# treangenlab/bronko

Hardware: AMD Instinct MI355X
Metric: reads/sec through call k-mer->pileup, SARS-CoV-2 k=21 (higher is better)
Workload: dtype u64

## Files before the change

bronko_amd/csrc/bk_finalize_lean.hip:

```cpp
#include <hip/hip_runtime.h>

#include "bk_device.h"
#include "bk_kernels.h"
#include "bk_scan_common.h"
#include "bk_finalize_common.h"

namespace bk {

constexpr int kLeanVBlock = 1024;
constexpr uint32_t kLeanVq = 64;
constexpr uint32_t kLeanWin = 256;

__device__ __forceinline__ void lean_vote(unsigned int* cnt, unsigned int* mxv, uint32_t span, uint32_t p0, const FinalizeArgs& a, uint32_t cell,
                                          uint32_t idx, bool canonical, uint64_t c, uint32_t isrc, int k, uint32_t v) {
    uint32_t bit_idx;
    bool forward;
    if (canonical) { bit_idx = ((uint32_t)(c >> (2 * idx)) & 3u) ^ 3u; forward = isrc != 0; }
    else { bit_idx = (uint32_t)(c >> (2 * (k - 1 - (int)idx))) & 3u; forward = isrc == 0; }
    const uint32_t pos = cell - p0;
    if (cell >= p0 && pos < span) {
        const uint32_t at = ((forward ? 0u : 4u) + bit_idx) * span + pos;
        __hip_atomic_fetch_add(cnt + at, 1u, __ATOMIC_RELAXED, __HIP_MEMORY_SCOPE_WORKGROUP);
        __hip_atomic_fetch_max(mxv + at, v, __ATOMIC_RELAXED, __HIP_MEMORY_SCOPE_WORKGROUP);
    } else {
        const size_t pc = (size_t)cell * 4 + bit_idx;
        atomicAdd(a.pileup + (forward ? 2 : 3) * a.plane + pc, 1ull);
        atomicMax(a.pileup + (forward ? 0 : 1) * a.plane + pc, (unsigned long long)v);
    }
}
__device__ __forceinline__ void lean_flush(const unsigned int* cnt, const unsigned int* mxv, uint32_t span, uint32_t p0, const FinalizeArgs& a) {
    for (uint32_t i = threadIdx.x; i < 8u * span; i += blockDim.x) {
        const unsigned int nv = cnt[i];
        if (!nv) continue;
        const uint32_t row = i / span, pos = i - row * span;
        const size_t pc = ((size_t)p0 + pos) * 4 + (row & 3u);
        atomicAdd(a.pileup + (row < 4u ? 2 : 3) * a.plane + pc, (unsigned long long)nv);
        atomicMax(a.pileup + (row < 4u ? 0 : 1) * a.plane + pc, (unsigned long long)mxv[i]);
    }
}

template <bool FUSED>
__global__ __launch_bounds__(kLeanVBlock) void finalize_vbin_kernel(FinalizeArgs a) {
    __shared__ unsigned int cnt[8 * kLeanWin], mxv[8 * kLeanWin];
    __shared__ uint32_t lstats[3 + 2];
    __shared__ unsigned int tmask[kLeanVq * kVRowsPerPos / 32 + 1];
    extern __shared__ __attribute__((aligned(16))) unsigned int acc[];
    const IndexView& ix = a.ix;
    const int k = ix.k;
    const uint32_t span = (uint32_t)ix.v_span, rl = span + 1u;
    const uint32_t q0 = blockIdx.x * kLeanVq;
    const uint32_t nq = ix.n_full + span;
    const uint32_t id_lo = min(q0 >= span - 1u ? q0 - (span - 1u) : 0u, ix.n_full - 1u);
    const uint32_t p0 = ix.id_rec[id_lo].cell;
    for (uint32_t i = threadIdx.x; i < 8u * kLeanWin; i += kLeanVBlock) { cnt[i] = 0u; mxv[i] = 0u; }
    if (threadIdx.x < 5) lstats[threadIdx.x] = 0u;
    if constexpr (FUSED) {
        const uint32_t n_eb = a.f_ig.n_ebins, n_bins = n_eb + a.f_ig.n_vbins, bin = n_eb + blockIdx.x, cap = a.f_ig.cap_v, G = a.f_ig.grid_max;
        const uint32_t upb = cap / 8u;
        const uint32_t vsize = kLeanVq * kVRowsPerPos * rl;
        const uint32_t n_units = a.f_n_wg * upb;
        const unsigned short* const bin_items = a.f_items + (size_t)n_eb * G * a.f_ig.cap_e + (size_t)blockIdx.x * G * cap;
        const bool mine = threadIdx.x < n_units;
        const uint32_t wg0 = mine ? threadIdx.x / upb : 0u, un0 = threadIdx.x - wg0 * upb;
        uint32_t hdr0 = 0u;
        uint4 v0 = make_uint4(0u, 0u, 0u, 0u);
        if (mine) { hdr0 = a.f_tab[(size_t)bin * G + wg0]; v0 = reinterpret_cast<const uint4*>(bin_items + (size_t)wg0 * cap)[un0]; }
        const unsigned long long ov_all = a.f_ov_n[a.f_ov_par];
        if (threadIdx.x <= kLeanVq * kVRowsPerPos / 32) {
            unsigned int* tw = a.f_touch + (size_t)blockIdx.x * (kLeanVq * kVRowsPerPos / 32) + threadIdx.x;
            unsigned int m = 0u;
            if (threadIdx.x < kLeanVq * kVRowsPerPos / 32) { m = *tw; if (m) *tw = 0u; }
            else m = ov_all > (unsigned long long)a.f_ov_cap ? 1u : 0u;
            tmask[threadIdx.x] = m;
        }
        for (uint32_t i = threadIdx.x; i < vsize; i += kLeanVBlock) acc[i] = 0u;
        __syncthreads();
        auto take = [&](uint32_t it) __attribute__((always_inline)) {
            __hip_atomic_fetch_add(acc + (it & 0x7fffu), (it & 0x8000u) ? 0u - 1u : 1u, __ATOMIC_RELAXED, __HIP_MEMORY_SCOPE_WORKGROUP);
        };
        auto take8 = [&](const uint4& v, uint32_t left) __attribute__((always_inline)) {
            if (left > 0u) take(v.x & 0xffffu);
            if (left > 1u) take(v.x >> 16);
            if (left > 2u) take(v.y & 0xffffu);
            if (left > 3u) take(v.y >> 16);
            if (left > 4u) take(v.z & 0xffffu);
            if (left > 5u) take(v.z >> 16);
            if (left > 6u) take(v.w & 0xffffu);
            if (left > 7u) take(v.w >> 16);
        };
        for (uint32_t u = threadIdx.x; u < n_units; u += kLeanVBlock) {
            const uint32_t wg = u / upb, un = u - wg * upb;
            uint32_t n_all; uint4 v;
            if (u == threadIdx.x) { n_all = hdr0; v = v0; }
            else { n_all = a.f_tab[(size_t)bin * G + wg]; v = reinterpret_cast<const uint4*>(bin_items + (size_t)wg * cap)[un]; }
            const uint32_t n = min(n_all, cap);
            take8(v, n > 8u * un ? n - 8u * un : 0u);
            const uint32_t g = min(n_all - n, kItemGCap);
            if (g) {
                const uint4* q = reinterpret_cast<const uint4*>(a.f_gext + ((size_t)wg * n_bins + bin) * kItemGCap);
                for (uint32_t i0 = 8u * un; i0 < g; i0 += 8u * upb * 4u) {
                    uint4 e[4];
#pragma unroll
                    for (uint32_t j = 0; j < 4u; ++j) e[j] = i0 + 8u * upb * j < g ? q[(i0 >> 3) + upb * j] : make_uint4(0u, 0u, 0u, 0u);
#pragma unroll
                    for (uint32_t j = 0; j < 4u; ++j) take8(e[j], g > i0 + 8u * upb * j ? g - i0 - 8u * upb * j : 0u);
                }
            }
        }
        {
            const uint32_t n_ov = (uint32_t)(ov_all < (unsigned long long)a.f_ov_cap ? ov_all : (unsigned long long)a.f_ov_cap);
            for (uint32_t i = threadIdx.x; i < n_ov; i += kLeanVBlock) {
                const uint32_t e = a.f_ov[i];
                if ((e >> 16) == bin) take(e & 0xffffu);
            }
        }
    }
    __syncthreads();
    unsigned long long* __restrict__ vc = const_cast<unsigned long long*>(a.counters) + ix.v_off;
    const uint32_t lpr = span, gpw = 64u / lpr;
    const uint32_t lane64 = threadIdx.x & 63u, wave = threadIdx.x >> 6;
    const uint32_t grp = lane64 / lpr, oo = lane64 - grp * lpr;
    const bool lane_on = grp < gpw;
    unsigned int kept = 0, distinct = 0, variant = 0;
    for (uint32_t g0 = 0; g0 < kLeanVq * kVRowsPerPos; g0 += (kLeanVBlock / 64) * gpw) {
        const uint32_t g = g0 + wave * gpw + grp;
        const uint32_t q = q0 + g / kVRowsPerPos, r6 = g % kVRowsPerPos;
        const bool in_row = lane_on && g < kLeanVq * kVRowsPerPos && q < nq;
        const size_t at = ((size_t)q * kVRowsPerPos + r6) * rl + oo;
        unsigned long long n;
        if constexpr (FUSED) {
            const uint32_t gg = in_row ? g : 0u;
            n = in_row ? (unsigned long long)(long long)(int32_t)acc[gg * rl + oo] : 0ull;
            if (in_row && (tmask[kLeanVq * kVRowsPerPos / 32] || ((tmask[gg >> 5] >> (gg & 31u)) & 1u))) {
                const unsigned long long pv = vc[at];
                if (pv) { n += pv; vc[at] = 0ull; }
            }
        } else {
            n = in_row ? vc[at] : 0ull;
            if (a.clear_v && n) vc[at] = 0ull;
        }
        const uint32_t d = r6 & 1u, alt = r6 >> 1;
        const bool inq = in_row && q >= oo && q - oo < ix.n_full;
        const uint32_t p = inq ? q - oo : 0u;
        const uint4 idr = *reinterpret_cast<const uint4*>(ix.id_rec + p);
        const uint64_t kmer_p = (uint64_t)idr.x | ((uint64_t)idr.y << 32);
        const uint32_t ambp = idr.w;
        const int o = (int)oo + ix.v_omin;
        if (!__ballot(n + (1ull << 26) >= (1ull << 27))) {
            int m = (int)(unsigned int)n;
#pragma unroll
            for (int off = 1; off < 32; off <<= 1) {
                const int t = __shfl_up(m, off, 64);
                if (oo >= (uint32_t)off) m += t;
            }
            n = (unsigned long long)(long long)m;
        } else {
#pragma unroll
            for (int off = 1; off < 32; off <<= 1) {
                const unsigned long long t = __shfl_up(n, off, 64);
                if (oo >= (uint32_t)off) n += t;
            }
        }
        bool act = inq && n != 0;
        const uint32_t rcid = (ambp >> 1) & 1u;
        const int j = rcid ? k - 1 - o : o;
        const int sh = 2 * (k - 1 - (act ? j : 0));
        const uint32_t bb = ((uint32_t)(kmer_p >> sh) & 3u) ^ (alt + 1u);
        const uint32_t isrc = d ^ rcid;
        const uint64_t c = (kmer_p & ~(3ull << sh)) | ((uint64_t)bb << sh);
        const uint64_t rc = revcomp_kmer(c, k);
        if (act && !(j >= ix.wstart && j < ix.wstart + ix.W && c < rc)) act = false;
        if (act) { distinct += 1; if (n < a.ci || n > a.cx) act = false; else kept += 1; }
        const uint32_t v = (uint32_t)(n > a.cs ? a.cs : n);
        bool defer = false;
        if (act) {
            bool plain = (ambp & kIdSimple) != 0u;
            if (plain && (ambp & 1u)) {
                const uint2 ans = *reinterpret_cast<const uint2*>(ix.dirty_ans + ans_index(p, (uint32_t)o, rcid ? 3u - bb : bb, k));
                plain = !(ans.y & (kAnsNone | kAnsMulti));
            }
            if (!plain) { defer = true; act = false; }
        }
        {
            const unsigned long long dm = __ballot(defer);
            if (dm) {
                unsigned int base = 0;
                if (lane64 == (uint32_t)__builtin_ctzll(dm)) base = atomicAdd(a.n_deferred, (unsigned int)__popcll(dm));
                base = (unsigned int)__shfl((int)base, __builtin_ctzll(dm));
                if (defer) {
                    const unsigned int slot = base + (unsigned int)__popcll(dm & ((1ull << lane64) - 1ull));
                    a.deferred[slot] = (uint32_t)at;
                    if (a.deferred_n) a.deferred_n[slot] = n;
                }
            }
        }
        if (act) lean_vote(cnt, mxv, kLeanWin, p0, a, idr.z + (uint32_t)j, (uint32_t)j, rcid != 0u, c, isrc, k, v);
        variant += act ? 1u : 0u;
    }
#pragma unroll
    for (int off = 32; off; off >>= 1) variant += (unsigned int)__shfl_xor((int)variant, off);
    if (lane64 == 0 && variant) atomicAdd(&lstats[1], variant);
    {
        const uint32_t W = (uint32_t)ix.W;
        const uint32_t sub = threadIdx.x & 15u, id = q0 + (threadIdx.x >> 4);
        unsigned int perfect = 0;
        if (id < ix.n_full) {
            const uint4 idr = *reinterpret_cast<const uint4*>(ix.id_rec + id);
            const unsigned long long n0 = a.counters[2 * (size_t)id], n1 = a.counters[2 * (size_t)id + 1];
            if (!(idr.w & kIdSimple)) {
                if (sub == 0u && (n0 | n1)) a.lean_e_list[atomicAdd(a.lean_n_list + 2, 1u)] = id;
            } else {
                const uint64_t km = (uint64_t)idr.x | ((uint64_t)idr.y << 32);
                const uint32_t rcid = (idr.w >> 1) & 1u;
#pragma unroll
                for (uint32_t isrc = 0; isrc < 2u; ++isrc) {
                    const unsigned long long n = isrc ? n1 : n0;
                    if (sub == 0u) distinct += n != 0;
                    if (n == 0 || n < a.ci || n > a.cx) continue;
                    if (sub == 0u) { kept += 1; perfect += 1; }
                    const uint32_t v = (uint32_t)(n > a.cs ? a.cs : n);
                    for (uint32_t t = sub; t < W; t += 16u) {
                        const uint32_t j = (uint32_t)ix.wstart + t;
                        lean_vote(cnt, mxv, kLeanWin, p0, a, idr.z + j, j, rcid != 0u, km, isrc, k, v);
                    }
                }
            }
        }
#pragma unroll
        for (int off = 32; off; off >>= 1) perfect += (unsigned int)__shfl_xor((int)perfect, off);
        if (lane64 == 0 && perfect) { atomicAdd(&lstats[0], perfect); atomicAdd(&lstats[2], perfect); }
    }
    __syncthreads();
    lean_flush(cnt, mxv, kLeanWin, p0, a);
    finalize_epilogue(a, lstats, kept, distinct, lstats + 3, (int)blockIdx.x);
}

bool finalize_lean_ok(const FinalizeArgs& a) {
    return !a.no_lean && a.lean_e_list && a.lean_n_list && !a.ix.slot_files && a.mode == 0 && !a.v_list && !a.p_list && !a.e_list && !a.ktab_keys && a.ix.n_prows == 0 && a.ix.n_u == a.ix.n_full &&
           a.ix.n_full > 0 && a.ix.n_files == 1 && a.ix.dirty_ans && a.ix.W > 1 && a.ix.v_span > 0 && a.ix.v_span <= 32 && a.partials && a.cs < (1ull << 32) &&
           a.elem_lo == 0 && a.elem_hi >= a.ix.v_off + v_plane_len(a.ix.n_full, a.ix.v_span, 0);
}
unsigned launch_finalize_lean_variant(const FinalizeArgs& a, hipStream_t stream) {
    const unsigned grid = (unsigned)((a.ix.n_full + (uint32_t)a.ix.v_span + kLeanVq - 1) / kLeanVq);
    if (a.f_items) {
        const size_t lds = (size_t)kLeanVq * kVRowsPerPos * ((size_t)a.ix.v_span + 1u) * sizeof(unsigned int);
        (void)raise_lds_limit(reinterpret_cast<const void*>(finalize_vbin_kernel<true>), lds + 20u * 1024u);
        hipLaunchKernelGGL(finalize_vbin_kernel<true>, dim3(grid), dim3(kLeanVBlock), lds, stream, a);
    } else {
        hipLaunchKernelGGL(finalize_vbin_kernel<false>, dim3(grid), dim3(kLeanVBlock), 0, stream, a);
    }
    return grid;
}
}
```

bronko_amd/csrc/bk_kernels.h:

```cpp
#pragma once
#include <hip/hip_runtime.h>

#include "../../include/bronko_hip.h"
#include "bk_device.h"

namespace bk {

struct ItemGeom {
    uint32_t n_ebins, n_vbins;
    uint32_t cap_e, cap_v;
    uint32_t vq_log2;
    uint32_t wg_items;
    uint32_t wg_stride;
    uint32_t grid_max;
};
constexpr uint32_t kEBinLog2 = 7;
constexpr uint32_t kERunMax = 255;
constexpr uint32_t kEBinSpan = (1u << kEBinLog2) + kERunMax;
constexpr uint32_t kItemGCap = 256;

struct ScanArgs {
    const IndexView* ixp;
    int32_t k, wstart, W, v_omin, v_span;
    uint64_t v_off;
// ... 21 lines not shown
    uint64_t n_records;
    const unsigned long long* n_records_dev;
    uint32_t stride_words;
    unsigned long long* counters;
    unsigned int* slabs;
    unsigned int* n_bits;
    unsigned int* n_any;
    unsigned int* l2_bits;
    unsigned int* l2_any;
    unsigned int* l2_plan;
    uint32_t l2_min_grid;
    uint2* l2_diag;
    uint32_t l2_words;
    uint32_t n_lds_bins;
    uint32_t win_lo;
    const uint32_t* win_dev;
    const uint32_t* occ;
    int32_t win_file, n_files;
    int ref_in_lds;
    unsigned long long* kmer_total;
    unsigned long long* ktab_keys;
    unsigned int* ktab_cnt;
    uint32_t ktab_log2;
    unsigned long long* ktab_overflow;
    uint32_t mate;
    unsigned int* touch_v;
    unsigned int* touch_b;
    unsigned int* touch_p;
    unsigned int* touch_e;
    unsigned long long rl_recip;
    ItemGeom ig;
    unsigned short* items;
    unsigned short* tab;
    unsigned short* gext;
    unsigned int* ov;
    unsigned long long* ov_n;
    uint32_t ov_cap;
    uint32_t ov_par;
    int n_direct;
    uint32_t stage_off;
    int ablate;
    unsigned long long* dbg;
};

struct FinalizeArgs {
    IndexView ix;
    const unsigned long long* counters;
    uint64_t elem_lo, elem_hi;
    unsigned long long ci, cs, cx;
    unsigned long long* pileup;
    size_t plane;
    unsigned long long* stats;
    unsigned char* present;
    unsigned long long* kept_total;
    unsigned long long* distinct_total;
    unsigned int* partials;
    int row_exact, row_general;
    const uint32_t* file_cell_lo;
    uint32_t max_file_cells;
    unsigned int* deferred;
    unsigned long long* deferred_n;
    int clear_v;
    unsigned int* deferred_mask;
    unsigned int* n_deferred;
    unsigned long long* ktab_keys;
    unsigned int* ktab_cnt;
    uint32_t ktab_log2;
    unsigned long long* ktab_overflow;
    uint32_t mate;
    const unsigned int* v_list;
    const unsigned int* p_list;
    const unsigned int* e_list;
    const unsigned int* n_list;
    int mode;
    const int* sel;
    int sel_file;
    unsigned int* lean_e_list;
    unsigned int* lean_n_list;
    int no_lean;
    const unsigned int* tail_e_list;
    const unsigned int* tail_n_list;
    unsigned long long* zero_e;
    size_t zero_e_n;
    int gather;
    int gather_ablate;
    unsigned long long* alias_hits;
    unsigned int* n_alias_hits;
    unsigned int alias_cap;
    const uint64_t* merged_slots;
    uint32_t n_merged_slots;
    const unsigned short* f_items;
    const unsigned short* f_tab;
    const unsigned short* f_gext;
    const unsigned int* f_ov;
    const unsigned long long* f_ov_n;
    uint32_t f_ov_cap, f_ov_par, f_n_wg;
    ItemGeom f_ig;
    unsigned int* f_touch;
};

struct FoldArgs {
    const unsigned int* slabs;
    uint32_t n_slabs;
    uint32_t n_lds_bins;
    const uint32_t* id_at;
    uint32_t win_lo;
    const uint32_t* win_dev;
    unsigned int* touch_e;
    const uint32_t* cell_codes;
    unsigned long long* counters;
};

struct PackArgs {
    const uint8_t* bases;
    uint32_t shift;
    const unsigned long long* offsets;
    uint64_t n_reads;
    int32_t k;
    uint32_t stride_words;
    uint32_t* words;
    uint16_t* lens;
    uint64_t cap;
    unsigned long long* n_records;
    unsigned long long* n_real;
    uint32_t* work;
};
struct QualArgs {
    const uint8_t* quals;
    uint32_t shift;
    uint32_t thr;
};
void launch_pack_reads(const PackArgs& a, unsigned long long* tally, hipStream_t stream, const QualArgs* q = nullptr, uint8_t* ends = nullptr);

constexpr uint32_t kEndFirst = 1u, kEndLast = 2u;
constexpr uint32_t kPrimerMinLen = BK_PRIMER_MIN_LEN, kPrimerMaxLen = BK_PRIMER_MAX_LEN, kMaxPrimers = BK_MAX_PRIMERS, kMaxPrimerMismatches = BK_PRIMER_MAX_MISMATCHES;
constexpr uint32_t kPrimerEntryWords = 9;
struct TrimArgs {
    uint32_t* words;
    uint16_t* lens;
    const uint8_t* ends;
    uint64_t n_records;
    const unsigned long long* n_records_dev;
    uint32_t stride_words;
    int32_t k;
    const uint32_t* table;
    uint32_t n_primers;
    uint32_t max_mismatches;
    unsigned long long* stats;
    unsigned long long* n_real;
};
void launch_primer_trim(const TrimArgs& a, int n_cus, hipStream_t stream);

constexpr uint32_t kAdapterMinLen = BK_ADAPTER_MIN_LEN, kAdapterMaxLen = BK_ADAPTER_MAX_LEN, kMaxAdapters = BK_MAX_ADAPTERS,
                   kAdapterMinOverlap = BK_ADAPTER_MIN_OVERLAP;
constexpr double kAdapterMaxErrorRate = BK_ADAPTER_MAX_ERROR_RATE;
static_assert(kAdapterMaxLen == 64 && kMaxAdapters <= 8, "AdapterEntry holds 64 bases, AdapterArgs eight entries");
constexpr uint32_t kNoCut = 0xFFFFFFFFu;
struct AdapterEntry {
    uint32_t code[4];
    uint32_t mask[4];
    uint32_t len;
    uint32_t allowed;
};
struct AdapterArgs {
    uint32_t* words;
    uint16_t* lens;
// ... 165 lines not shown
```

bronko_amd/csrc/bk_kernels.hip:

```cpp
#include <hip/hip_runtime.h>

#include <algorithm>
#include <cstdlib>
#include <mutex>
#include <utility>
#include <vector>

#include "bk_device.h"
#include "bk_kernels.h"
#include "bk_scan_common.h"
#include "bk_finalize_common.h"

namespace bk {


__device__ __forceinline__ int probe_table(const TableSlot* __restrict__ sub, uint32_t log2s, uint64_t key) {
    const uint32_t smask = (1u << log2s) - 1u;
    uint32_t h = hash_key(key, log2s);
    for (;;) {
        const uint4 e = *reinterpret_cast<const uint4*>(sub + h);
        const uint64_t kk = (uint64_t)e.x | ((uint64_t)e.y << 32);
        if (kk == key) return (int)e.z;
        if (kk == kEmptyKey) return -1;
        h = (h + 1) & smask;
// ... 1734 lines not shown
__global__ __launch_bounds__(256) void fold_kernel(FoldArgs f) {
    const uint64_t tid = (uint64_t)blockIdx.x * 256 + threadIdx.x;
    const uint64_t nthreads = (uint64_t)gridDim.x * 256;
    const uint32_t per = (f.n_slabs + gridDim.y - 1) / gridDim.y;
    const uint32_t b0 = blockIdx.y * per, b1 = min(f.n_slabs, b0 + per);
    for (uint64_t i = tid; i < f.n_lds_bins && b0 < b1; i += nthreads) {
        unsigned long long s0 = 0, s1 = 0;
        for (uint32_t b = b0; b < b1; ++b) {
            const unsigned int v = f.slabs[(size_t)b * f.n_lds_bins + i];
            s0 += v & 0xffffu;
            s1 += v >> 16;
        }
        if (s0 | s1) {
            const uint64_t cell = (f.win_dev ? f.win_dev[1] : f.win_lo) + i;
            const uint32_t id = f.id_at[cell];
            const uint32_t rc = ((f.cell_codes[cell >> 4] >> (2 * (cell & 15))) & 3u) == 2u ? 1u : 0u;
            touch(f.touch_e, id);
            if (s0) atomicAdd(f.counters + 2 * (size_t)id + rc, s0);
            if (s1) atomicAdd(f.counters + 2 * (size_t)id + (1u - rc), s1);
        }
    }
}

void launch_fold(const FoldArgs& f, hipStream_t stream) {
    const uint64_t work = f.n_lds_bins;
    if (work == 0) return;
    uint64_t blocks = (work + 255) / 256;
    if (blocks > 1024) blocks = 1024;
    const unsigned groups = std::max(1u, std::min(8u, f.n_slabs / 8));
    hipLaunchKernelGGL(fold_kernel, dim3((unsigned)blocks, groups), dim3(256), 0, stream, f);
}

__device__ __forceinline__ uint32_t first_of_file(const DevEntry* __restrict__ ent, uint32_t cnt, int file) {
    uint32_t lo = 0, hi = cnt;
    while (lo < hi) {
        const uint32_t mid = (lo + hi) >> 1;
        if ((int)ent[mid].file < file) lo = mid + 1; else hi = mid;
    }
    return lo;
}

template <int B>
__device__ __forceinline__ void write_lane(int& acc, int nb) { asm("v_writelane_b32 %0, %1, %2" : "+v"(acc) : "s"(nb), "n"(B)); }
template <int... B>
__device__ __forceinline__ void tally_word(uint32_t wd, int& acc, std::integer_sequence<int, B...>) {
    (write_lane<B>(acc, __popcll(__ballot((wd & (1u << B)) != 0u))), ...);
}
template <bool ATOMIC, uint32_t COL = 1u>
__device__ __forceinline__ void tally_files(const uint4& fb, uint32_t* lstats, uint32_t lane, uint32_t n_files) {
    if (!__ballot(files_any(fb))) return;
#pragma unroll
    for (uint32_t w = 0; w < 4u; ++w) {
        const uint32_t wd = w == 0u ? fb.x : w == 1u ? fb.y : w == 2u ? fb.z : fb.w;
        if (w * 32u >= n_files || !__ballot(wd != 0u)) continue;
        int acc = 0;
        tally_word(wd, acc, std::make_integer_sequence<int, 32>{});
        const uint32_t f = w * 32u + lane;
        if (lane < 32u && acc && f < n_files) {
            if (ATOMIC) atomicAdd(&lstats[f * 3u + COL], (uint32_t)acc); else lstats[f * 3u + COL] += (uint32_t)acc;
        }
    }
}

__global__ __launch_bounds__(256) void finalize_reduce_kernel(FinalizeArgs a, int n_rows, unsigned long long* zero_p, size_t zero_n) {
    __shared__ unsigned long long wave_sums[4];
    const int n3 = a.ix.n_files * 3, cols = n3 + 2;
    for (size_t i = (size_t)blockIdx.x * 256 + threadIdx.x; i < zero_n; i += (size_t)gridDim.x * 256) zero_p[i] = 0ull;
    if (a.lean_n_list && blockIdx.x == 0 && threadIdx.x < 8) a.lean_n_list[threadIdx.x] = 0u;
    const int col = blockIdx.x;
    unsigned long long s = 0;
    for (int r = threadIdx.x; r < n_rows; r += 256) s += a.partials[(size_t)r * cols + col];
#pragma unroll
    for (int off = 32; off; off >>= 1) s += __shfl_xor(s, off);
    if ((threadIdx.x & 63) == 0) wave_sums[threadIdx.x >> 6] = s;
    __syncthreads();
    if (threadIdx.x != 0) return;
    s = wave_sums[0] + wave_sums[1] + wave_sums[2] + wave_sums[3];
    if (!s) return;
    if (col < n3) { a.stats[col] += s; if (col % 3 != 2) a.present[col / 3] = 1; }
    else if (col == n3) { if (a.kept_total) *a.kept_total += s; }
    else if (a.distinct_total) *a.distinct_total += s;
}

constexpr int kVoteSlots = 512;
constexpr uint32_t kVoteMaxEntries = 4;
constexpr size_t kVoteLdsBytes = (size_t)kVoteSlots * (8 + 8 + 4 + 2) + 16;
struct VoteTable {
    unsigned long long* keys;
    unsigned long long* mx;
    unsigned int* cnt;
    unsigned int* n_used;
    unsigned short* used;
};
__device__ __forceinline__ VoteTable vt_make(unsigned char* lds) {
    VoteTable vt;
    vt.keys = reinterpret_cast<unsigned long long*>(lds);
    vt.mx = vt.keys + kVoteSlots;
    vt.cnt = reinterpret_cast<unsigned int*>(vt.mx + kVoteSlots);
    vt.n_used = vt.cnt + kVoteSlots;
    vt.used = reinterpret_cast<unsigned short*>(vt.n_used + 4);
    return vt;
}
__device__ __forceinline__ void vt_clear(const VoteTable& vt) {
    for (int i = threadIdx.x; i < kVoteSlots; i += blockDim.x) { vt.keys[i] = ~0ull; vt.mx[i] = 0ull; vt.cnt[i] = 0u; }
    if (threadIdx.x == 0) { vt.n_used[0] = 0u; vt.n_used[1] = 0u; }
}
__device__ __forceinline__ void vt_vote(const VoteTable& vt, uint32_t par, const FinalizeArgs& a, const DevEntry& e, uint64_t c, uint32_t isrc,
                                        int k, unsigned long long v) {
    if (a.mode == 1 || (a.mode == 2 && (int)e.file != a.sel_file)) return;
    uint32_t bit_idx;
    bool forward;
    if (e.canonical) { bit_idx = ((uint32_t)(c >> (2 * e.idx)) & 3u) ^ 3u; forward = isrc != 0; }
    else { bit_idx = (uint32_t)(c >> (2 * (k - 1 - e.idx))) & 3u; forward = isrc == 0; }
    const unsigned long long key = (((unsigned long long)e.cell * 4 + bit_idx) << 1) | (forward ? 0ull : 1ull);
    uint32_t h = (uint32_t)((key * 0x9E3779B97F4A7C15ull) >> 55) & (kVoteSlots - 1);
    for (int probe = 0; probe < 8; ++probe) {
        const unsigned long long old = atomicCAS(&vt.keys[h], ~0ull, key);
        if (old == ~0ull) vt.used[atomicAdd(vt.n_used + par, 1u)] = (unsigned short)h;
        if (old == ~0ull || old == key) { atomicAdd(&vt.cnt[h], 1u); atomicMax(&vt.mx[h], v); return; }
        h = (h + 1) & (kVoteSlots - 1);
    }
    vote(a, e, c, isrc, k, v);
}
__device__ __forceinline__ void vt_flush(const VoteTable& vt, uint32_t par, const FinalizeArgs& a) {
    __syncthreads();
    const unsigned int nu = vt.n_used[par];
    if (threadIdx.x == 0) vt.n_used[par ^ 1u] = 0u;
    for (unsigned int u = threadIdx.x; u < nu; u += blockDim.x) {
        const int i = vt.used[u];
        const unsigned long long key = vt.keys[i];
        const size_t cell = (size_t)(key >> 1);
        atomicAdd(a.pileup + ((key & 1ull) ? 3 : 2) * a.plane + cell, (unsigned long long)vt.cnt[i]);
        atomicMax(a.pileup + ((key & 1ull) ? 1 : 0) * a.plane + cell, vt.mx[i]);
        vt.keys[i] = ~0ull; vt.mx[i] = 0ull; vt.cnt[i] = 0u;
    }
    __syncthreads();
    if (threadIdx.x == 0) { vt.n_used[0] = 0u; vt.n_used[1] = 0u; }
}

__device__ __forceinline__ void v_kmer_of_counter(const IndexView& ix, const unsigned long long* __restrict__ vc, uint64_t vi,
                                                  uint32_t& p, uint32_t& t, uint64_t& c, uint32_t& isrc, unsigned long long& n) {
    const int k = ix.k;
    const uint64_t real_len = v_real_len(ix.n_full, ix.v_span);
    uint32_t bb;
    if (vi < real_len) {
        const uint32_t rl = (uint32_t)ix.v_span + 1u;
        const uint64_t row = vi / rl;
        const uint32_t oo = (uint32_t)(vi % rl);
        n = 0;
        if (vc) for (uint32_t x = 0; x <= oo; ++x) n += vc[row * rl + x];
        const uint32_t r6 = (uint32_t)(row % kVRowsPerPos);
        p = (uint32_t)(row / kVRowsPerPos) - oo;
        const uint32_t rcid = (ix.amb[p] >> 1) & 1u;
        const int o = (int)oo + ix.v_omin;
        const int j = rcid ? k - 1 - o : o;
        const uint32_t own = (uint32_t)(ix.kmer_of[p] >> (2 * (k - 1 - j))) & 3u;
        bb = own ^ ((r6 >> 1) + 1u);
        isrc = (r6 & 1u) ^ rcid;
        t = (uint32_t)(j - ix.wstart);
    } else {
        const uint64_t x = vi - real_len;
        isrc = (uint32_t)x & 1u;
        bb = (uint32_t)(x >> 1) & 3u;
        p = ix.prow_id[x >> 3];
        t = ix.prow_t[x >> 3];
        n = vc ? vc[vi] : 0ull;
// ... 662 lines not shown
            v = v > a.cs ? a.cs : v;

            int s = -1;
            if (lane < ix.W) {
                if (ci < n_e) {
                    s = (int)ix.slot_of[(size_t)(ci >> 1) * ix.W + lane];
                } else {
                    const int sh = 2 * (k - 1 - (ix.wstart + lane));
                    s = probe_table(ix.table + (size_t)lane * S, ix.log2s, c & ~(3ull << sh));
                }
            }
            if (a.mode == 1) note_alias(s, c, isrc, v);
            for (unsigned long long bm = __ballot(s >= 0); bm; bm &= bm - 1ull) {
                const int sb = __shfl(s, __builtin_ctzll(bm));
                const uint32_t off = ix.ent_off[sb], cnt = ix.ent_len[sb];
                for (uint32_t q = (uint32_t)lane; q < cnt; q += 64u) {
                    const DevEntry e = ix.entries[off + q];
                    if (atomicAdd(&hits[e.file], 1u) == 0u) touched[atomicAdd(ntouched, 1u)] = e.file;
                    vote(a, e, c, isrc, k, v);
                }
            }
            __syncthreads();
            const uint32_t nt = *ntouched;
            uint32_t n_perfect = 0;
            int my_perfect = -1;
            for (uint32_t q = lane; q < ((nt + 63u) & ~63u); q += 64) {
                bool perfect = false;
                if (q < nt) {
                    const uint32_t g = touched[q];
                    const uint32_t h = hits[g];
                    hits[g] = 0;
                    perfect = h == (uint32_t)ix.W;
                    if (do_stats) lstats[g * 3 + (perfect ? 0 : 1)] += 1;
                    if (perfect) my_perfect = (int)g;
                }
                n_perfect += (uint32_t)__popcll(__ballot(perfect));
            }
            if (do_stats && n_perfect == 1 && my_perfect >= 0) lstats[my_perfect * 3 + 2] += 1;
            __syncthreads();
            if (lane == 0) *ntouched = 0;
            __syncthreads();
        }
    };
    if (a.mode == 1 && ix.ent_files) {
        for (uint64_t item0 = (uint64_t)blockIdx.x * 64; item0 < n_items; item0 += (uint64_t)gridDim.x * 64) {
            const uint64_t item = item0 + (uint32_t)lane;
            const bool on = item < n_items;
            unsigned long long v = 0;
            uint64_t c = 0;
            uint32_t isrc = 0, p_ = 0, t_ = 0;
            if (on) v_kmer_of_counter(ix, nullptr, a.deferred[item], p_, t_, c, isrc, v);
            uint4 acc = make_uint4(0u, 0u, 0u, 0u);
            uint32_t found = 0, alias_n = 0;
            int alias_sb = -1;
            bool generic = false;
            for (int t = 0; t < ix.W; ++t) {
                const int sh = 2 * (k - 1 - (ix.wstart + t));
                const int sb = on ? probe_table(ix.table + (size_t)t * S, ix.log2s, c & ~(3ull << sh)) : -1;
                if (sb < 0) continue;
                const uint4 fb = ix.ent_files[sb];
                generic |= !files_any(fb);
                acc.x |= fb.x; acc.y |= fb.y; acc.z |= fb.z; acc.w |= fb.w;
                found |= 1u << t;
                alias_sb = (a.alias_hits && ix.slot_alias && ((ix.slot_alias[(uint32_t)sb >> 5] >> ((uint32_t)sb & 31u)) & 1u)) ? (alias_n++ ? -2 : sb) : alias_sb;
            }
            generic |= found == 0xffffffffu >> (32 - ix.W);
            generic |= alias_sb == -2;
            if (on && !generic && alias_sb >= 0) {
                unsigned long long n_; uint64_t c2; uint32_t i2, p2, t2;
                v_kmer_of_counter(ix, a.counters + ix.v_off, a.deferred[item], p2, t2, c2, i2, n_);
                note_alias(alias_sb, c, isrc, n_);
            }
            if (on && a.deferred_mask) a.deferred_mask[item] = found;
            if (!on || generic) acc = make_uint4(0u, 0u, 0u, 0u);
            tally_files<false>(acc, lstats, (uint32_t)lane, (uint32_t)ix.n_files);
            for (unsigned long long gm = __ballot(on && generic); gm; gm &= gm - 1ull) wave_item(item0 + (uint64_t)__builtin_ctzll(gm));
        }
    } else
    for (uint64_t item = blockIdx.x; item < n_items + n_tail; item += gridDim.x) wave_item(item);
    __syncthreads();
    if (lane == 0) { ntouched[0] = 0; ntouched[1] = 0; }
    __syncthreads();
    if (do_stats) finalize_epilogue(a, lstats, tail_kept, tail_distinct, ntouched, a.row_general + (int)blockIdx.x);
}

__global__ __launch_bounds__(256) void compact_touched_kernel(unsigned int* bm, uint64_t n_bits, unsigned int* list, unsigned int* n_out,
                                                              uint64_t split, uint64_t cap) {
    const uint64_t n_words = (n_bits + 31) / 32;
    const int lane = threadIdx.x & 63;
    for (uint64_t w0 = (uint64_t)blockIdx.x * 256; w0 < n_words; w0 += (uint64_t)gridDim.x * 256) {
        const uint64_t w = w0 + threadIdx.x;
        const uint32_t bits = w < n_words ? bm[w] : 0u;
        if (!__ballot(bits != 0u)) continue;
        if (bits) bm[w] = 0u;
        const uint32_t lo_mask = w * 32 + 32 <= split ? ~0u : w * 32 >= split ? 0u : (1u << (uint32_t)(split - w * 32)) - 1u;
        uint32_t lo = bits & lo_mask, hi = bits & ~lo_mask;
        const uint32_t n_lo = (uint32_t)__popc(lo), n_hi = (uint32_t)__popc(hi);
        uint32_t inc = n_lo | (n_hi << 16);
#pragma unroll
        for (int d = 1; d < 64; d <<= 1) { const uint32_t up = (uint32_t)__shfl_up((int)inc, d); if (lane >= d) inc += up; }
        uint32_t base_lo = 0, base_hi = 0;
        if (lane == 63) {
            if (inc & 0xffffu) base_lo = atomicAdd(n_out, inc & 0xffffu);
            if (inc >> 16) base_hi = atomicAdd(n_out + 1, inc >> 16);
        }
        base_lo = (uint32_t)__shfl((int)base_lo, 63) + (inc & 0xffffu) - n_lo;
        base_hi = (uint32_t)__shfl((int)base_hi, 63) + (inc >> 16) - n_hi;
        for (; lo; lo &= lo - 1u) list[base_lo++] = (uint32_t)(w * 32) + (uint32_t)__builtin_ctz(lo);
        for (; hi; hi &= hi - 1u) list[cap - 1 - base_hi++] = (uint32_t)(w * 32) + (uint32_t)__builtin_ctz(hi);
    }
}
__global__ __launch_bounds__(256) void expand_touched_blocks_kernel(unsigned int* touch_b, uint32_t n_blocks, const uint2* cell_blk, unsigned int* touch_v,
                                                                    uint32_t span, uint64_t n_q) {
    const uint32_t gb = blockIdx.x * 4u + (threadIdx.x >> 6), lane = threadIdx.x & 63u;
    if (gb >= n_blocks || !((touch_b[gb >> 5] >> (gb & 31u)) & 1u)) return;
    if (lane == 0) atomicAnd(touch_b + (gb >> 5), ~(1u << (gb & 31u)));
    const long long q_0 = (long long)gb * 64 + (long long)(int32_t)cell_blk[gb].x;
    const long long q_lo = max(q_0 - (long long)span, 0ll);
    const long long q_hi = min(q_0 + 64 + (long long)span, (long long)n_q);
    if (q_lo >= q_hi) return;
    const uint64_t r0 = (uint64_t)q_lo * kVRowsPerPos, r1 = (uint64_t)q_hi * kVRowsPerPos;
    for (uint64_t w = (r0 >> 5) + lane; w * 32u < r1; w += 64u) {
        const uint64_t lo = max(w * 32u, r0), hi = min(w * 32u + 32u, r1);
        const uint32_t take = (uint32_t)(hi - lo);
        atomicOr(touch_v + w, (take == 32u ? 0xffffffffu : (1u << take) - 1u) << (uint32_t)(lo & 31u));
    }
}
void launch_expand_touched_blocks(unsigned int* touch_b, uint32_t n_blocks, const uint2* cell_blk, unsigned int* touch_v, uint32_t span, uint64_t n_q, hipStream_t stream) {
    if (!n_blocks) return;
    hipLaunchKernelGGL(expand_touched_blocks_kernel, dim3((n_blocks + 3u) / 4u), dim3(256), 0, stream, touch_b, n_blocks, cell_blk, touch_v, span, n_q);
}
void launch_compact_touched(unsigned int* touch_v, uint64_t n_rows, unsigned int* touch_p, uint64_t n_prows, unsigned int* touch_e, uint64_t n_ids,
                            uint64_t n_full, unsigned int* v_list, unsigned int* p_list, unsigned int* e_list, unsigned int* n_list, hipStream_t stream) {
    auto go = [&](unsigned int* bm, uint64_t n, unsigned int* list, unsigned int* cnt, uint64_t split) {
        if (!n) return;
        const uint64_t blocks = std::max<uint64_t>(1, std::min<uint64_t>(((n + 31) / 32 + 255) / 256, 2048));
        hipLaunchKernelGGL(compact_touched_kernel, dim3((unsigned)blocks), dim3(256), 0, stream, bm, n, list, cnt, split, n);
    };
    go(touch_v, n_rows, v_list, n_list + 0, ~0ull);
    go(touch_p, n_prows, p_list, n_list + 4, ~0ull);
    go(touch_e, n_ids, e_list, n_list + 2, n_full);
}
__global__ __launch_bounds__(256) void clear_touched_kernel(unsigned long long* counters, uint64_t v_off, uint64_t v_real, uint32_t rl,
                                                            const unsigned int* v_list, const unsigned int* p_list, const unsigned int* e_list,
                                                            const unsigned int* n_list, uint64_t n_ids) {
    const uint64_t t = (uint64_t)blockIdx.x * 256 + threadIdx.x, nt = (uint64_t)gridDim.x * 256;
    unsigned long long* vc = counters + v_off;
    for (uint64_t i = t; i < (uint64_t)n_list[0] * rl; i += nt) vc[(uint64_t)v_list[i / rl] * rl + i % rl] = 0ull;
    for (uint64_t i = t; i < (uint64_t)n_list[4] * 8ull; i += nt) vc[v_real + (uint64_t)p_list[i >> 3] * 8ull + (i & 7ull)] = 0ull;
    for (uint64_t i = t; i < (uint64_t)n_list[2] * 2ull; i += nt) counters[2ull * e_list[i >> 1] + (i & 1ull)] = 0ull;
    for (uint64_t i = t; i < (uint64_t)n_list[3] * 2ull; i += nt) counters[2ull * e_list[n_ids - 1 - (i >> 1)] + (i & 1ull)] = 0ull;
}
void launch_clear_touched(unsigned long long* counters, uint64_t v_off, uint64_t v_real_len, uint32_t rl, const unsigned int* v_list,
                          const unsigned int* p_list, const unsigned int* e_list, const unsigned int* n_list, uint64_t n_ids, hipStream_t stream) {
    hipLaunchKernelGGL(clear_touched_kernel, dim3(2048), dim3(256), 0, stream, counters, v_off, v_real_len, rl, v_list, p_list, e_list, n_list, n_ids);
}

size_t finalize_lds_bytes(int n_files) { return ((size_t)n_files * 5 + 4) * sizeof(uint32_t); }
constexpr unsigned kFinVariantBlocks = 256 * 8, kFinExactBlocks = 256 * 8, kFinGeneralBlocks = 256 * 32;
size_t finalize_partial_rows() { return (size_t)kFinVariantBlocks + kFinExactBlocks + kFinGeneralBlocks; }

static unsigned finalize_general_blocks(const FinalizeArgs& a) {
    return (unsigned)std::min<size_t>(a.ix.n_files >= 8 ? kFinGeneralBlocks : kFinGeneralBlocks / 32, 256 * std::max<size_t>(1, (160u * 1024u) / finalize_lds_bytes(a.ix.n_files)));
}
bool finalize_runs_by_region(const FinalizeArgs& a) {
    return finalize_lean_ok(a) && (uint64_t)(a.ix.n_full + (uint32_t)a.ix.v_span) / 64 + (uint64_t)a.ix.total_cells / 256 + 2 + 64 + finalize_general_blocks(a) <= finalize_partial_rows();
}
void launch_finalize(const FinalizeArgs& a0, hipStream_t stream) {
    if (a0.ix.W <= 0) return;
    FinalizeArgs a = a0;
    const size_t lds_stats = ((size_t)a.ix.n_files * 3 + 2) * sizeof(uint32_t);
    const uint64_t rows_per_group = 4ull * (64ull / (uint64_t)std::max(a.ix.v_span, 1));
    const uint64_t n_v = std::max<uint64_t>((v_real_rows(a.ix.n_full, a.ix.v_span) + rows_per_group - 1) / rows_per_group * 256ull, a.ix.n_prows * 8ull);
    const unsigned b_var = (unsigned)std::max<uint64_t>(1, std::min<uint64_t>((n_v + 255) / 256, kFinVariantBlocks));
    const size_t lds_votes = (lds_stats + 15) / 16 * 16 + kVoteLdsBytes;
    const size_t lds = finalize_lds_bytes(a.ix.n_files);
    if (lds_votes > 64 * 1024 || lds > 64 * 1024) {
        (void)hipFuncSetAttribute(reinterpret_cast<const void*>(finalize_variant_kernel<false>), hipFuncAttributeMaxDynamicSharedMemorySize, (int)lds_votes);
        (void)hipFuncSetAttribute(reinterpret_cast<const void*>(finalize_variant_kernel<true>), hipFuncAttributeMaxDynamicSharedMemorySize, (int)lds_votes);
        (void)hipFuncSetAttribute(reinterpret_cast<const void*>(finalize_exact_kernel), hipFuncAttributeMaxDynamicSharedMemorySize, (int)lds_votes);
        (void)hipFuncSetAttribute(reinterpret_cast<const void*>(finalize_general_kernel), hipFuncAttributeMaxDynamicSharedMemorySize, (int)lds);
    }
    const unsigned b_gen = finalize_general_blocks(a);
    if (a.gather && a.mode >= 2) {
        if (a.ix.n_prows) {
            if (a.ix.slot_files) hipLaunchKernelGGL(finalize_variant_kernel<true>, dim3(64), dim3(256), lds_votes, stream, a);
            else hipLaunchKernelGGL(finalize_variant_kernel<false>, dim3(64), dim3(256), lds_votes, stream, a);
        }
        if (a.ix.n_u > a.ix.n_full) hipLaunchKernelGGL(finalize_exact_kernel, dim3(64), dim3(256), lds_votes, stream, a);
        if (a.alias_hits) launch_alias_votes(a, stream);
        return;
    }
    unsigned b_v = b_var, b_e = 0;
    const bool lean = finalize_runs_by_region(a);
    if (lean) {
        b_v = launch_finalize_lean_variant(a, stream);
        a.tail_e_list = a.lean_e_list; a.tail_n_list = a.lean_n_list;
        b_e = 0;
    } else {
    if (a.ix.slot_files) hipLaunchKernelGGL(finalize_variant_kernel<true>, dim3(b_var), dim3(256), lds_votes, stream, a);
    else hipLaunchKernelGGL(finalize_variant_kernel<false>, dim3(b_var), dim3(256), lds_votes, stream, a);
    const uint64_t n_work = e_plane_len(a.ix.n_u) * (uint64_t)a.ix.W;
    const unsigned b_ex = (unsigned)std::max<uint64_t>(1, std::min<uint64_t>((n_work + 255) / 256, kFinExactBlocks));
    a.row_exact = (int)b_var;
    if (a.mode == 2 && a.file_cell_lo && a.ix.id_own_files && a.max_file_cells)
        hipLaunchKernelGGL(finalize_exact_own_kernel, dim3((a.max_file_cells + kOwnCells - 1) / kOwnCells), dim3(256), 0, stream, a);
    else if (a.mode == 0 && a.e_list && a.file_cell_lo && a.ix.id_own_files && a.ix.cell_file && a.ix.estat_files && a.ix.id_rest_off && a.ix.total_cells)
        hipLaunchKernelGGL(finalize_exact_own_kernel, dim3((a.ix.total_cells + kOwnCells - 1) / kOwnCells), dim3(256), 0, stream, a);
    hipLaunchKernelGGL(finalize_exact_kernel, dim3(b_ex), dim3(256), lds_votes, stream, a);
    b_e = b_ex;
    }
    a.row_general = (int)(b_v + b_e);
    hipLaunchKernelGGL(finalize_general_kernel, dim3(b_gen), dim3(64), lds, stream, a);
    if (a.partials && a.mode < 2) {
        const int cols = a.ix.n_files * 3 + 2;
        hipLaunchKernelGGL(finalize_reduce_kernel, dim3((unsigned)cols), dim3(256), 0, stream, a, (int)(b_v + b_e + b_gen), a.zero_e, a.zero_e_n);
    }
}

__global__ __launch_bounds__(256) void zero_small_kernel(unsigned long long* a, size_t na, unsigned long long* b, size_t nb, unsigned long long* c, size_t nc,
                                                         unsigned char* d, size_t nd, unsigned int* e, size_t ne, unsigned long long* big, size_t nbig) {
    const size_t t = (size_t)blockIdx.x * blockDim.x + threadIdx.x, n = (size_t)gridDim.x * blockDim.x;
    for (size_t i = t; i < na; i += n) a[i] = 0;
    for (size_t i = t; i < nb; i += n) b[i] = 0;
    for (size_t i = t; i < nc; i += n) c[i] = 0;
    for (size_t i = t; i < nd; i += n) d[i] = 0;
    for (size_t i = t; i < ne; i += n) e[i] = 0;
    ulonglong2* big2 = reinterpret_cast<ulonglong2*>(big);
    for (size_t i = t; i < nbig / 2; i += n) big2[i] = make_ulonglong2(0ull, 0ull);
    if (t == 0 && (nbig & 1)) big[nbig - 1] = 0;
}
void launch_zero_small(unsigned long long* a, size_t na, unsigned long long* b, size_t nb, unsigned long long* c, size_t nc,
                       unsigned char* d, size_t nd, unsigned int* e, size_t ne, unsigned long long* big, size_t nbig, hipStream_t stream) {
    const unsigned grid = (unsigned)std::max<size_t>(16, std::min<size_t>((nbig / 2 + 255) / 256, 2048));
    hipLaunchKernelGGL(zero_small_kernel, dim3(grid), dim3(256), 0, stream, a, na, b, nb, c, nc, d, nd, e, ne, big, nbig);
}

__global__ void pack_sums_kernel(unsigned long long* sums, const unsigned long long* stats, const unsigned char* present,
                                 const unsigned long long* kstats, int n_files, unsigned long long* xflag) {
    const int n_s = 2 * n_files * 3, n_p = 2 * n_files;
    for (int i = blockIdx.x * blockDim.x + threadIdx.x; i < n_s + n_p + 9; i += gridDim.x * blockDim.x)
        sums[i] = i < n_s ? stats[i] : i < n_s + n_p ? (unsigned long long)present[i - n_s] : i < n_s + n_p + 8 ? kstats[i - n_s - n_p] : xflag[0];
}
__global__ void unpack_sums_kernel(const unsigned long long* sums, unsigned long long* stats, unsigned char* present,
                                   unsigned long long* kstats, int n_files, unsigned long long* xflag) {
    const int n_s = 2 * n_files * 3, n_p = 2 * n_files;
    for (int i = blockIdx.x * blockDim.x + threadIdx.x; i < n_s + n_p + 9; i += gridDim.x * blockDim.x) {
        if (i < n_s) stats[i] = sums[i];
        else if (i < n_s + n_p) present[i - n_s] = sums[i] ? 1 : 0;
        else if (i < n_s + n_p + 8) kstats[i - n_s - n_p] = sums[i];
        else { if (sums[i]) xflag[1] = 1ull; xflag[0] = 0ull; }
    }
}
void launch_pack_sums(unsigned long long* sums, const unsigned long long* stats, const unsigned char* present, const unsigned long long* kstats,
                      int n_files, unsigned long long* xflag, hipStream_t stream) {
    hipLaunchKernelGGL(pack_sums_kernel, dim3(8), dim3(256), 0, stream, sums, stats, present, kstats, n_files, xflag);
}
void launch_unpack_sums(const unsigned long long* sums, unsigned long long* stats, unsigned char* present, unsigned long long* kstats,
                        int n_files, unsigned long long* xflag, hipStream_t stream) {
    hipLaunchKernelGGL(unpack_sums_kernel, dim3(8), dim3(256), 0, stream, sums, stats, present, kstats, n_files, xflag);
}

struct XportGeom {
    uint64_t plane_len, part_len, v_off;
    uint32_t n_parts;
    uint64_t part_elems;
};
BK_HD uint64_t xport_e_in_part(const XportGeom& g, uint64_t p) {
    const uint64_t lo = p * g.part_len;
    return g.v_off > lo ? (g.v_off - lo < g.part_len ? g.v_off - lo : g.part_len) : 0ull;
}
__global__ __launch_bounds__(256) void xport_measure_kernel(const unsigned long long* __restrict__ plane, XportGeom g, unsigned long long* out ) {
    unsigned long long me = 0, mv = 0;
    for (uint64_t i = (uint64_t)blockIdx.x * 256 + threadIdx.x; i < g.plane_len; i += (uint64_t)gridDim.x * 256) {
        const unsigned long long v = plane[i];
        if (i < g.v_off) me = max(me, v);
        else { const long long sv = (long long)v; mv = max(mv, (unsigned long long)(sv < 0 ? -sv : sv)); }
    }
#pragma unroll
    for (int off = 32; off; off >>= 1) { me = max(me, (unsigned long long)__shfl_xor(me, off)); mv = max(mv, (unsigned long long)__shfl_xor(mv, off)); }
    if ((threadIdx.x & 63) == 0) { if (me) atomicMax(out, me); if (mv) atomicMax(out + 1, mv); }
}
template <int WIDTH>
__global__ __launch_bounds__(256) void xport_pack_kernel(const unsigned long long* __restrict__ plane, XportGeom g, void* buf, unsigned long long* flag) {
    bool bad = false;
    for (uint64_t i = (uint64_t)blockIdx.x * 256 + threadIdx.x; i < g.plane_len; i += (uint64_t)gridDim.x * 256) {
        const uint64_t p = i / g.part_len, j = i - p * g.part_len;
        const unsigned long long v = plane[i];
        const long long sv = (long long)v;
        if (WIDTH == 32) {
            bad |= sv > (long long)(0x7fffffffll / g.n_parts) || sv < -(long long)(0x7fffffffll / g.n_parts);
            static_cast<int*>(buf)[p * g.part_elems + j] = (int)sv;
        } else {
            const uint64_t n_e = xport_e_in_part(g, p);
            unsigned short* part = static_cast<unsigned short*>(buf) + p * g.part_elems;
            const long long lim = 32767 / g.n_parts;
            if (j < n_e) {
// ... 60 lines not shown
```

Baseline: 8.674 billion.

## Stage id records in LDS and fold final reduce into general kernel tail

The lean variant kernel now loads its window of id records and the per-id exact counters into shared memory once, instead of re-reading global memory inside the vote and exact loops. It also clears simple-id exact counters inline. Separately, the last finishing block of the general finalize kernel, chosen by an atomic ticket, now does the partials reduction and tail zeroing, which removes the separate reduce kernel launch on the lean path. The cost is extra LDS use, a serial 64-lane reduction in one block, and reliance on fence and ticket ordering.

New measurement: 8.077 billion. -6.9%, worse.

```diff
diff --git a/bronko_amd/csrc/bk_finalize_lean.hip b/bronko_amd/csrc/bk_finalize_lean.hip
--- a/bronko_amd/csrc/bk_finalize_lean.hip
+++ b/bronko_amd/csrc/bk_finalize_lean.hip
@@ -10,6 +10,7 @@
 constexpr int kLeanVBlock = 1024;
 constexpr uint32_t kLeanVq = 64;
 constexpr uint32_t kLeanWin = 256;
+constexpr uint32_t kLeanRecs = kLeanVq + 32;
 
 __device__ __forceinline__ void lean_vote(unsigned int* cnt, unsigned int* mxv, uint32_t span, uint32_t p0, const FinalizeArgs& a, uint32_t cell,
                                           uint32_t idx, bool canonical, uint64_t c, uint32_t isrc, int k, uint32_t v) {
@@ -44,6 +45,8 @@
     __shared__ unsigned int cnt[8 * kLeanWin], mxv[8 * kLeanWin];
     __shared__ uint32_t lstats[3 + 2];
     __shared__ unsigned int tmask[kLeanVq * kVRowsPerPos / 32 + 1];
+    __shared__ uint4 recs[kLeanRecs];
+    __shared__ unsigned long long ecnt[2 * kLeanVq];
     extern __shared__ __attribute__((aligned(16))) unsigned int acc[];
     const IndexView& ix = a.ix;
     const int k = ix.k;
@@ -51,7 +54,17 @@
     const uint32_t q0 = blockIdx.x * kLeanVq;
     const uint32_t nq = ix.n_full + span;
     const uint32_t id_lo = min(q0 >= span - 1u ? q0 - (span - 1u) : 0u, ix.n_full - 1u);
-    const uint32_t p0 = ix.id_rec[id_lo].cell;
+    const uint32_t st = kLeanVBlock - 1u - threadIdx.x, st_e = st - kLeanRecs;
+    const uint32_t id_hi = min(q0 + kLeanVq, ix.n_full);
+    const bool st_rec = st < kLeanRecs && id_lo + st < id_hi, st_cnt = st_e < 2u * kLeanVq && q0 + (st_e >> 1) < ix.n_full;
+    uint4 st_r = make_uint4(0u, 0u, 0u, 0u);
+    unsigned long long st_n = 0ull;
+    if (st_rec) st_r = *reinterpret_cast<const uint4*>(ix.id_rec + id_lo + st);
+    if (st_cnt) st_n = a.counters[2 * (size_t)q0 + st_e];
+    auto stage = [&]() __attribute__((always_inline)) {
+        if (st < kLeanRecs) recs[st] = st_r;
+        if (st_e < 2u * kLeanVq) ecnt[st_e] = st_n;
+    };
     for (uint32_t i = threadIdx.x; i < 8u * kLeanWin; i += kLeanVBlock) { cnt[i] = 0u; mxv[i] = 0u; }
     if (threadIdx.x < 5) lstats[threadIdx.x] = 0u;
     if constexpr (FUSED) {
@@ -74,6 +87,7 @@
             tmask[threadIdx.x] = m;
         }
         for (uint32_t i = threadIdx.x; i < vsize; i += kLeanVBlock) acc[i] = 0u;
+        stage();
         __syncthreads();
         auto take = [&](uint32_t it) __attribute__((always_inline)) {
             __hip_atomic_fetch_add(acc + (it & 0x7fffu), (it & 0x8000u) ? 0u - 1u : 1u, __ATOMIC_RELAXED, __HIP_MEMORY_SCOPE_WORKGROUP);
@@ -114,8 +128,12 @@
                 if ((e >> 16) == bin) take(e & 0xffffu);
             }
         }
+    } else {
+        stage();
     }
     __syncthreads();
+    const uint32_t p0 = recs[0].z;
+    if (a.zero_e && st_cnt && st_n && (recs[q0 + (st_e >> 1) - id_lo].w & kIdSimple)) a.zero_e[2 * (size_t)q0 + st_e] = 0ull;
     unsigned long long* __restrict__ vc = const_cast<unsigned long long*>(a.counters) + ix.v_off;
     const uint32_t lpr = span, gpw = 64u / lpr;
     const uint32_t lane64 = threadIdx.x & 63u, wave = threadIdx.x >> 6;
@@ -142,7 +160,7 @@
         const uint32_t d = r6 & 1u, alt = r6 >> 1;
         const bool inq = in_row && q >= oo && q - oo < ix.n_full;
         const uint32_t p = inq ? q - oo : 0u;
-        const uint4 idr = *reinterpret_cast<const uint4*>(ix.id_rec + p);
+        const uint4 idr = recs[inq ? p - id_lo : 0u];
         const uint64_t kmer_p = (uint64_t)idr.x | ((uint64_t)idr.y << 32);
         const uint32_t ambp = idr.w;
         const int o = (int)oo + ix.v_omin;
@@ -205,8 +223,8 @@
         const uint32_t sub = threadIdx.x & 15u, id = q0 + (threadIdx.x >> 4);
         unsigned int perfect = 0;
         if (id < ix.n_full) {
-            const uint4 idr = *reinterpret_cast<const uint4*>(ix.id_rec + id);
-            const unsigned long long n0 = a.counters[2 * (size_t)id], n1 = a.counters[2 * (size_t)id + 1];
+            const uint4 idr = recs[id - id_lo];
+            const unsigned long long n0 = ecnt[2u * (threadIdx.x >> 4)], n1 = ecnt[2u * (threadIdx.x >> 4) + 1u];
             if (!(idr.w & kIdSimple)) {
                 if (sub == 0u && (n0 | n1)) a.lean_e_list[atomicAdd(a.lean_n_list + 2, 1u)] = id;
             } else {
diff --git a/bronko_amd/csrc/bk_kernels.h b/bronko_amd/csrc/bk_kernels.h
--- a/bronko_amd/csrc/bk_kernels.h
+++ b/bronko_amd/csrc/bk_kernels.h
@@ -127,6 +127,7 @@
     const unsigned int* tail_n_list;
     unsigned long long* zero_e;
     size_t zero_e_n;
+    int fold_rows;
     int gather;
     int gather_ablate;
     unsigned long long* alias_hits;
diff --git a/bronko_amd/csrc/bk_kernels.hip b/bronko_amd/csrc/bk_kernels.hip
--- a/bronko_amd/csrc/bk_kernels.hip
+++ b/bronko_amd/csrc/bk_kernels.hip
@@ -1840,6 +1840,39 @@
     else if (a.distinct_total) *a.distinct_total += s;
 }
 
+__device__ __forceinline__ void finalize_fold_reduce(const FinalizeArgs& a, uint64_t n_tail) {
+    const uint32_t lane = threadIdx.x;
+    unsigned int* const ticket = a.lean_n_list + 7;
+    __syncthreads();
+    unsigned int drawn = 0;
+    if (lane == 0) drawn = __hip_atomic_fetch_add(ticket, 1u, __ATOMIC_RELEASE, __HIP_MEMORY_SCOPE_AGENT);
+    drawn = (unsigned int)__shfl((int)drawn, 0);
+    if (drawn != gridDim.x - 1u) return;
+    __builtin_amdgcn_fence(__ATOMIC_ACQUIRE, "agent");
+    constexpr uint32_t cols = 5;
+    unsigned long long s[cols] = {0ull, 0ull, 0ull, 0ull, 0ull};
+    const uint32_t n_words = (uint32_t)a.fold_rows * cols;
+    for (uint32_t i = lane; i < n_words; i += 64u) {
+        const unsigned long long v = a.partials[i];
+        const uint32_t c = i % cols;
+#pragma unroll
+        for (uint32_t j = 0; j < cols; ++j) s[j] += c == j ? v : 0ull;
+    }
+#pragma unroll
+    for (uint32_t j = 0; j < cols; ++j) {
+#pragma unroll
+        for (int off = 32; off; off >>= 1) s[j] += __shfl_xor(s[j], off);
+    }
+    if (lane == 0) {
+#pragma unroll
+        for (uint32_t j = 0; j < 3u; ++j) if (s[j]) { a.stats[j] += s[j]; if (j != 2u) a.present[0] = 1; }
+        if (s[3] && a.kept_total) *a.kept_total += s[3];
+        if (s[4] && a.distinct_total) *a.distinct_total += s[4];
+    }
+    if (a.zero_e) for (uint64_t i = lane; i < n_tail; i += 64u) a.zero_e[2ull * a.tail_e_list[i >> 1] + (i & 1ull)] = 0ull;
+    if (lane < 8u) a.lean_n_list[lane] = 0u;
+}
+
 constexpr int kVoteSlots = 512;
 constexpr uint32_t kVoteMaxEntries = 4;
 constexpr size_t kVoteLdsBytes = (size_t)kVoteSlots * (8 + 8 + 4 + 2) + 16;
@@ -2668,6 +2701,7 @@
     if (lane == 0) { ntouched[0] = 0; ntouched[1] = 0; }
     __syncthreads();
     if (do_stats) finalize_epilogue(a, lstats, tail_kept, tail_distinct, ntouched, a.row_general + (int)blockIdx.x);
+    if (a.fold_rows) finalize_fold_reduce(a, n_tail);
 }
 
 __global__ __launch_bounds__(256) void compact_touched_kernel(unsigned int* bm, uint64_t n_bits, unsigned int* list, unsigned int* n_out,
@@ -2783,6 +2817,7 @@
         b_v = launch_finalize_lean_variant(a, stream);
         a.tail_e_list = a.lean_e_list; a.tail_n_list = a.lean_n_list;
         b_e = 0;
+        a.fold_rows = (int)(b_v + b_gen);
     } else {
     if (a.ix.slot_files) hipLaunchKernelGGL(finalize_variant_kernel<true>, dim3(b_var), dim3(256), lds_votes, stream, a);
     else hipLaunchKernelGGL(finalize_variant_kernel<false>, dim3(b_var), dim3(256), lds_votes, stream, a);
@@ -2798,7 +2833,7 @@
     }
     a.row_general = (int)(b_v + b_e);
     hipLaunchKernelGGL(finalize_general_kernel, dim3(b_gen), dim3(64), lds, stream, a);
-    if (a.partials && a.mode < 2) {
+    if (a.partials && a.mode < 2 && !a.fold_rows) {
         const int cols = a.ix.n_files * 3 + 2;
         hipLaunchKernelGGL(finalize_reduce_kernel, dim3((unsigned)cols), dim3(256), 0, stream, a, (int)(b_v + b_e + b_gen), a.zero_e, a.zero_e_n);
     }
```
